# zhangganlin/vista-slam

Hardware: AMD Instinct MI355X
Metric: STA image-pairs/sec @512x384 (higher is better)
Workload: dtype f16x3-split MFMA (3 fp16 products) in the transformer and the pose head; fp16 MFMA + one block-scaled fp8 correction MFMA in the DPT head's convolutions; fp32 accumulate; 1 GPU; 512x384 batch=8 pairs/GPU STA two-view forward (BASELINE configs[1]); pairs_per_gpu=8, H=384, W=512, precision=f16x3h, parallelism=single GPU

## Files before the change

vista_slam_amd/csrc/gemm2.h:

```cpp
#pragma once
#include "gemm.h"
#include <type_traits>

typedef short short8 __attribute__((ext_vector_type(8)));

__device__ __forceinline__ void glds16(const void* gsrc, void* lds_dst_wave_base) {
    __builtin_amdgcn_global_load_lds((const __attribute__((address_space(1))) void*)gsrc,
                                     (__attribute__((address_space(3))) void*)lds_dst_wave_base, 16, 0, 0);
}

template <bool SPLIT, int BM, int BN>
constexpr int gemm2_smem_bytes(int nstg = 2) { return nstg * (SPLIT ? 2 : 1) * (BM + BN) * 64; }

template <bool SPLIT>
__device__ __forceinline__ int lds2_off(int row, int chunk) {
    return SPLIT ? row * 128 + ((chunk ^ ((row >> 1) & 7)) << 4) : row * 64 + ((chunk ^ ((row >> 2) & 3)) << 4);
}

template <int BM, int MT, int NT, int WM, int WAVES_N>
__device__ __forceinline__ void head_epilogue(const GemmParams& p, const floatx16 (&acc)[MT][NT], int64_t pix_base, int rstride, int rows_valid,
                                              int cols_valid, int wm, int wn, int tid, char* smem) {
    float* red = reinterpret_cast<float*>(smem);
    const int lane = tid & 63, l31 = lane & 31, lhi = lane >> 5;
    float bv[NT], w4[NT][4];
#pragma unroll
    for (int j = 0; j < NT; ++j) {
        const int col = (wn * NT + j) * 32 + l31;
        bv[j] = p.bias ? p.bias[col] : 0.f;
#pragma unroll
        for (int o = 0; o < 4; ++o) w4[j][o] = p.hw4[o * 128 + col];
    }
    __syncthreads();
#pragma unroll
    for (int i = 0; i < MT; ++i) {
        float part[64];
#pragma unroll
        for (int r = 0; r < 16; ++r) {
#pragma unroll
            for (int j = 0; j < NT; ++j) {
                const float v = fmaxf(acc[i][j][r] + bv[j], 0.f);
#pragma unroll
                for (int o = 0; o < 4; ++o) part[r * 4 + o] = j == 0 ? v * w4[j][o] : __builtin_fmaf(v, w4[j][o], part[r * 4 + o]);
            }
        }
#pragma unroll
        for (int m = 16, n = 64; m >= 1; m >>= 1, n >>= 1) {
            const bool up = (l31 & m) != 0;
#pragma unroll
            for (int k = 0; k < 32; ++k) {
                if (k < n / 2) {
                    const float send = up ? part[k] : part[k + n / 2];
                    const float keep = up ? part[k + n / 2] : part[k];
                    part[k] = keep + __shfl_xor(send, m);
                }
            }
        }
        const int r = l31 >> 1, row = wm * WM + i * 32 + (r & 3) + 8 * (r >> 2) + 4 * lhi;
        *reinterpret_cast<float2*>(red + ((size_t)wn * BM + row) * 4 + (l31 & 1) * 2) = make_float2(part[0], part[1]);
    }
    __syncthreads();
    if (tid < BM) {
        const int64_t pix = pix_base + (int64_t)(tid >> 5) * rstride + (tid & 31);
        if (pix < p.M && (tid >> 5) < rows_valid && (tid & 31) < cols_valid) {
            float4 a = *reinterpret_cast<const float4*>(red + (size_t)tid * 4);
#pragma unroll
            for (int w = 1; w < WAVES_N; ++w) {
                const float4 b = *reinterpret_cast<const float4*>(red + ((size_t)w * BM + tid) * 4);
                a.x += b.x; a.y += b.y; a.z += b.z; a.w += b.w;
            }
            const float x = a.x + p.hb4[0], y = a.y + p.hb4[1], z = a.z + p.hb4[2], c = a.w + p.hb4[3];
            const float d = sqrtf(x * x + y * y + z * z);
            const float sc = expm1f(d) / fmaxf(d, 1e-8f);
            const bool second = pix >= p.hsplit;
            const int64_t q = second ? pix - p.hsplit : pix;
            float* pts = (second ? p.hptsB : p.hptsA) + q * 3;
            pts[0] = x * sc; pts[1] = y * sc; pts[2] = z * sc;
            (second ? p.hconfB : p.hconfA)[q] = 1.0f + expf(c);
        }
    }
}

template <int BM, int MT, int WM, int WAVES_N>
__device__ __forceinline__ void head_epilogue_t(const GemmParams& p, const floatx16 (&acc)[MT][1], int64_t pix_base, int rstride, int rows_valid,
                                                int cols_valid, int wm, int wn, int tid, char* smem) {
    float* red = reinterpret_cast<float*>(smem);
    const int lane = tid & 63, l31 = lane & 31, lhi = lane >> 5;
    float bv[16];
#pragma unroll
    for (int r = 0; r < 16; ++r) bv[r] = p.bias ? p.bias[wn * 32 + (r & 3) + 8 * (r >> 2) + 4 * lhi] : 0.f;
    half8 wh[2], wl[2];
    {
        RangeAcc rw;
#pragma unroll
        for (int w = 0; w < 2; ++w)
#pragma unroll
            for (int e = 0; e < 8; ++e) {
                const float x = l31 < 4 ? p.hw4[l31 * 128 + wn * 32 + 16 * w + 8 * lhi + e] * p.hw4_scale[l31 & 3] : 0.f;
                f16 h_, l_; split_f16(x, h_, l_, rw);
                wh[w][e] = h_; wl[w][e] = l_;
            }
    }
    __syncthreads();
    RangeAcc ra;
#pragma unroll
    for (int i = 0; i < MT; ++i) {
        floatx16 o;
#pragma unroll
        for (int r = 0; r < 16; ++r) o[r] = 0.f;
#pragma unroll
        for (int w = 0; w < 2; ++w) {
            union { half8 h; unsigned u[4]; } ph, pl;
#pragma unroll
            for (int e = 0; e < 8; ++e) {
                const float v = fmaxf(acc[i][0][8 * w + e] + bv[8 * w + e], 0.f);
                f16 h_, l_; split_f16(v, h_, l_, ra);
                ph.h[e] = h_; pl.h[e] = l_;
            }
#pragma unroll
            for (int e = 0; e < 2; ++e) {
                auto r1 = __builtin_amdgcn_permlane32_swap(ph.u[e], ph.u[2 + e], false, false);
                ph.u[e] = r1[0]; ph.u[2 + e] = r1[1];
                auto r2 = __builtin_amdgcn_permlane32_swap(pl.u[e], pl.u[2 + e], false, false);
                pl.u[e] = r2[0]; pl.u[2 + e] = r2[1];
            }
            o = __builtin_amdgcn_mfma_f32_32x32x16_f16(wl[w], ph.h, o, 0, 0, 0);
            o = __builtin_amdgcn_mfma_f32_32x32x16_f16(wh[w], pl.h, o, 0, 0, 0);
            o = __builtin_amdgcn_mfma_f32_32x32x16_f16(wh[w], ph.h, o, 0, 0, 0);
        }
        if (lhi == 0) *reinterpret_cast<float4*>(red + ((size_t)wn * BM + wm * WM + i * 32 + l31) * 4) =
            make_float4(o[0] / p.hw4_scale[0], o[1] / p.hw4_scale[1], o[2] / p.hw4_scale[2], o[3] / p.hw4_scale[3]);
    }
    ra.flush(p.range);
    __syncthreads();
    if (tid < BM) {
        const int64_t pix = pix_base + (int64_t)(tid >> 5) * rstride + (tid & 31);
        if (pix < p.M && (tid >> 5) < rows_valid && (tid & 31) < cols_valid) {
            float4 a = *reinterpret_cast<const float4*>(red + (size_t)tid * 4);
#pragma unroll
            for (int w = 1; w < WAVES_N; ++w) {
                const float4 b = *reinterpret_cast<const float4*>(red + ((size_t)w * BM + tid) * 4);
                a.x += b.x; a.y += b.y; a.z += b.z; a.w += b.w;
            }
            const float x = a.x + p.hb4[0], y = a.y + p.hb4[1], z = a.z + p.hb4[2], c = a.w + p.hb4[3];
            const float d = sqrtf(x * x + y * y + z * z);
            const float sc = expm1f(d) / fmaxf(d, 1e-8f);
            const bool second = pix >= p.hsplit;
            const int64_t q = second ? pix - p.hsplit : pix;
            float* pts = (second ? p.hptsB : p.hptsA) + q * 3;
            pts[0] = x * sc; pts[1] = y * sc; pts[2] = z * sc;
            (second ? p.hconfB : p.hconfA)[q] = 1.0f + expf(c);
        }
    }
}

template <bool SPLIT, int EPI, int NW, bool MX = false>
__device__ __forceinline__ void gemm2_tail(const GemmParams& p, const int tb, char* smem) {
    const int tid = threadIdx.x, lane = tid & 63, l31 = lane & 31, lhi = lane >> 5;
    const int wave = __builtin_amdgcn_readfirstlane(tid >> 6);
    constexpr int A_ES = SPLIT ? 64 : 32;
    const int row0 = p.M - p.m_tail, col0 = tb * 32;
    const int arow = row0 + l31 < p.M ? row0 + l31 : p.M - 1;
    const int brow = col0 + l31 < p.N ? col0 + l31 : p.N - 1;
    const f16* ap = p.A_hi + (size_t)arow * A_ES + lhi * 8;
    const f16* bp = p.B_hi + (size_t)brow * 64 + lhi * 8;
    const size_t a_kstride = (size_t)p.a_rp * A_ES, b_kstride = (size_t)p.N * 64;
    const int nkt_all = p.K / GEMM_BK;
    const int kt0 = (int)((int64_t)wave * nkt_all / NW), kt1 = (int)((int64_t)(wave + 1) * nkt_all / NW);
    struct Frag { uint4 ah[2], al[2], bh[2], bl[2]; };
    auto load = [&](int kt, Frag& f) {
        const f16* a = ap + kt * a_kstride;
        const f16* b = bp + kt * b_kstride;
#pragma unroll
        for (int ks = 0; ks < 2; ++ks) {
            f.ah[ks] = ldg16(a + ks * 16); f.bh[ks] = ldg16(b + ks * 16);
            if (MX) {
                f.al[ks] = ldg16(a - lhi * 8 + 32 + lhi * 16 + ks * 8); f.bl[ks] = ldg16(b - lhi * 8 + 32 + lhi * 16 + ks * 8);
            } else if (SPLIT) { f.al[ks] = ldg16(a + 32 + ks * 16); f.bl[ks] = ldg16(b + 32 + ks * 16); }
        }
    };
    floatx16 acc;
#pragma unroll
    for (int r = 0; r < 16; ++r) acc[r] = 0.f;
    auto mma = [&](const Frag& f) {
        if constexpr (MX) {
            typedef int int8v __attribute__((ext_vector_type(8)));
            union U8 { struct { uint4 x, y; } q; int8v v; } a8, b8;
#pragma unroll
            for (int ks = 0; ks < 2; ++ks) {
                H8 ah, bh; ah.u = f.ah[ks]; bh.u = f.bh[ks];
                acc = __builtin_amdgcn_mfma_f32_32x32x16_f16(ah.h, bh.h, acc, 0, 0, 0);
            }
            a8.q.x = f.al[0]; a8.q.y = f.al[1]; b8.q.x = f.bl[0]; b8.q.y = f.bl[1];
            constexpr int sc_a = 127 - STA_MX_A_SLO, sc_b = 127 - STA_MX_W_SHI;
            acc = __builtin_amdgcn_mfma_scale_f32_32x32x64_f8f6f4(a8.v, b8.v, acc, 1 , 0 , 0, sc_a, 0, sc_b);
            return;
        }
#pragma unroll
        for (int ks = 0; ks < 2; ++ks) {
            H8 ah, al, bh, bl; ah.u = f.ah[ks]; bh.u = f.bh[ks];
            if (SPLIT) {
                al.u = f.al[ks]; bl.u = f.bl[ks];
                acc = __builtin_amdgcn_mfma_f32_32x32x16_f16(al.h, bh.h, acc, 0, 0, 0);
                acc = __builtin_amdgcn_mfma_f32_32x32x16_f16(ah.h, bl.h, acc, 0, 0, 0);
            }
            acc = __builtin_amdgcn_mfma_f32_32x32x16_f16(ah.h, bh.h, acc, 0, 0, 0);
        }
    };
#pragma unroll 1
    for (int kt = kt0; kt < kt1; ++kt) {
        Frag f;
        load(kt, f);
        mma(f);
    }
    float* red = reinterpret_cast<float*>(smem);
#pragma unroll
    for (int r = 0; r < 16; ++r) red[(wave * 16 + r) * 64 + lane] = acc[r];
    __syncthreads();
    if (wave != 0) return;
#pragma unroll 1
    for (int w = 1; w < NW; ++w) {
#pragma unroll
        for (int r = 0; r < 16; ++r) acc[r] += red[(w * 16 + r) * 64 + lane];
    }
    epilogue_tile<SPLIT, EPI>(p, acc, row0, col0 + l31, lane, 0);
}

#ifndef STA_RING_ABL
#define STA_RING_ABL 0
#endif
template <bool SPLIT, int AMODE, int EPI, int BM, int BN, int WAVES_M, int WAVES_N, int ABL_ = 0, int NSTG = 2, bool MX = false>
__device__ __forceinline__ void gemm2_body(const GemmParams& p, const int block_id_in) {
    constexpr int ABL = ABL_ | (NSTG > 2 ? STA_RING_ABL : 0);
    extern __shared__ __attribute__((aligned(16))) char smem[];
    constexpr int NW = WAVES_M * WAVES_N;
    constexpr int WM = BM / WAVES_M, WN = BN / WAVES_N, MT = WM / 32, NT = WN / 32;
    constexpr int RB = SPLIT ? 128 : 64;
    constexpr int RPS = 1024 / RB;
    constexpr int CPR = RB / 16;
    constexpr int A_TILE = BM * RB, B_TILE = BN * RB, STAGE = A_TILE + B_TILE;
    constexpr int NSA = BM / RPS, NSB = BN / RPS;
    constexpr int SA = (NSA + NW - 1) / NW, SB = (NSB + NW - 1) / NW;
    constexpr int A_ES = SPLIT ? 64 : 32;
    static_assert(BM % 32 == 0 && BN % 32 == 0 && WM % 32 == 0 && WN % 32 == 0, "tile/wave mismatch");
    constexpr bool TRN = EPI == EPI_HEAD && BN == 128 && NT == 1;

    int block_id = block_id_in;
    constexpr bool HAS_TAIL = AMODE == A_DENSE && NSTG == 2 && ABL_ == 0 && BM >= 192 &&
                              (EPI == EPI_F32 || EPI == EPI_F32R || ((EPI == EPI_GELU || EPI == EPI_QKV) && !MX));
    if constexpr (HAS_TAIL) {
        if (p.m_tail > 0) {
            const int ntail = (p.N + 31) >> 5;
            if (block_id < ntail) { gemm2_tail<SPLIT, EPI, NW, MX>(p, block_id, smem); return; }
            block_id -= ntail;
        }
    }
    const int tid = threadIdx.x, lane = tid & 63;
    const int wave = __builtin_amdgcn_readfirstlane(tid >> 6);
    const int wm = wave / WAVES_N, wn = wave % WAVES_N;
    const int l31 = lane & 31, lhi = lane >> 5;
    unsigned long long clk0 = 0, rt0 = 0;
    if (p.clk_dbg) { clk0 = __builtin_readcyclecounter(); rt0 = __builtin_amdgcn_s_memrealtime(); }
    unsigned long long st0 = 0, st1 = 0, st2 = 0;
    if (p.stamps) st0 = __builtin_amdgcn_s_memrealtime();

    const int tiles_m = (p.M - (HAS_TAIL ? p.m_tail : 0) + BM - 1) / BM, tiles_n = (p.N + BN - 1) / BN;
    const int ksplit = p.ksplit > 1 ? p.ksplit : 1;
    const int nwg = tiles_m * tiles_n * ksplit;
    int t;
    {
        const int bid = block_id, q = nwg / 8, r = nwg % 8, xcd = bid % 8;
        t = (xcd < r ? xcd * (q + 1) : r * (q + 1) + (xcd - r) * q) + bid / 8;
    }
    const int kslice = t % ksplit;
    t /= ksplit;
    int bm, bn;
    {
        const int band = t / (4 * tiles_n);
        const int hb = tiles_m - band * 4 < 4 ? tiles_m - band * 4 : 4;
        const int local = t - band * 4 * tiles_n;
        bm = band * 4 + local % hb;
        bn = local / hb;
    }
    const int m0 = bm * BM, n0 = bn * BN;

    const int row_in = lane / CPR, c_lds = lane % CPR;
    unsigned a_src[SA], b_src[SB];
    int cv_pix0[SA]; unsigned cv_mask[SA], cv_coff[SA];
#pragma unroll
    for (int s = 0; s < SA; ++s) {
        const int row = RPS * (wave + NW * s) + row_in;
        const int sw = SPLIT ? (row >> 1) & 7 : (row >> 2) & 3;
        const int chunk = c_lds ^ sw;
        const int gm = m0 + row;
        if (AMODE == A_DENSE) {
            const int gmc = gm < p.M ? gm : p.M - 1;
            a_src[s] = ((unsigned)gmc * A_ES + chunk * 8) * 2u;
        } else {
            const bool rok = gm < p.M;
            const int gmc = rok ? gm : 0;
            const int hw = p.Ho * p.Wo;
            const int img = gmc / hw;
            const int rem = gmc - img * hw;
            const int y0 = (rem / p.Wo) * p.cstride - 1, x0 = (rem % p.Wo) * p.cstride - 1;
            cv_pix0[s] = (img * p.Hi + y0) * p.Wi + x0;
            unsigned mk = 0;
#pragma unroll
            for (int t = 0; t < 9; ++t) {
                const int yi = y0 + t / 3, xi = x0 + t % 3;
                if (rok && yi >= 0 && yi < p.Hi && xi >= 0 && xi < p.Wi) mk |= 1u << t;
            }
            cv_mask[s] = mk;
            cv_coff[s] = (unsigned)chunk * 16u;
            a_src[s] = 0;
        }
    }
#pragma unroll
    for (int s = 0; s < SB; ++s) {
        const int row = RPS * (wave + NW * s) + row_in;
        const int sw = SPLIT ? (row >> 1) & 7 : (row >> 2) & 3;
        const int gn = n0 + row;
        const int gnc = gn < p.N ? gn : p.N - 1;
        b_src[s] = ((unsigned)gnc * 64 + (c_lds ^ sw) * 8) * 2u;
    }
    const size_t a_kstride = (size_t)p.a_rp * A_ES, b_kstride = (size_t)p.N * 64;

    int cv_tap = 0, cv_cb = 0;
    const char* a_run = nullptr; const char* b_run = nullptr;
    auto issue_tile = [&](int kt, int stage) {
        char* sA = smem + stage * STAGE;
        char* sB = sA + A_TILE;
        int tap_off = 0; const char* a_cb = nullptr;
        if (AMODE == A_CONV3) {
            const int ky = cv_tap >= 6 ? 2 : (cv_tap >= 3 ? 1 : 0), kx = cv_tap - 3 * ky;
            tap_off = ky * p.Wi + kx;
            a_cb = reinterpret_cast<const char*>(p.A_hi) + (size_t)cv_cb * p.a_rp * (A_ES * 2);
        }
#pragma unroll
        for (int s = 0; s < SA; ++s) {
            if (NSA % NW != 0 && wave + NW * s >= NSA) continue;
            char* dst = sA + (wave + NW * s) * 1024;
            if (AMODE == A_DENSE) {
                unsigned o = a_src[s];
                asm volatile("" : "+v"(o));
                glds16(a_run + o, dst);
            } else {
                const unsigned off = (unsigned)(cv_pix0[s] + tap_off) * (unsigned)(A_ES * 2) + cv_coff[s];
                const bool ok = (cv_mask[s] >> cv_tap) & 1u;
                glds16(ok ? static_cast<const void*>(a_cb + off) : static_cast<const void*>(p.zero_page), dst);
            }
        }
        if (AMODE == A_CONV3) { if (++cv_cb == (p.Cin >> 5)) { cv_cb = 0; ++cv_tap; } }
#pragma unroll
        for (int s = 0; s < SB; ++s) {
            if (NSB % NW != 0 && wave + NW * s >= NSB) continue;
            unsigned o = b_src[s];
            asm volatile("" : "+v"(o));
            glds16(b_run + o, sB + (wave + NW * s) * 1024);
        }
        a_run += a_kstride * 2; b_run += b_kstride * 2;
    };

    floatx16 acc[MT][NT];
#pragma unroll
    for (int i = 0; i < MT; ++i)
#pragma unroll
        for (int j = 0; j < NT; ++j)
#pragma unroll
            for (int r = 0; r < 16; ++r) acc[i][j][r] = 0.f;

    const int nkt_all = p.K / GEMM_BK;
    const int kt0 = (int)((int64_t)kslice * nkt_all / ksplit);
    const int nkt = (int)((int64_t)(kslice + 1) * nkt_all / ksplit) - kt0;
    if (AMODE == A_CONV3) { const int cblocks = p.Cin >> 5; cv_tap = kt0 / cblocks; cv_cb = kt0 - cv_tap * cblocks; }
    a_run = reinterpret_cast<const char*>(p.A_hi + kt0 * a_kstride); b_run = reinterpret_cast<const char*>(p.B_hi + kt0 * b_kstride);
    constexpr bool RING = NSTG > 2;
    constexpr int GPW = SA + SB;
    static_assert(!RING || (NSA % NW == 0 && NSB % NW == 0), "ring needs the same DMA count in every wave");
    static_assert(NSTG >= 2 && NSTG <= 5, "2..5 stages");
    if (RING) {
#pragma unroll
        for (int s0 = 0; s0 < NSTG - 1; ++s0)
            if (s0 < nkt && !(ABL & 1)) issue_tile(kt0 + s0, s0);
    } else {
        issue_tile(kt0, 0);
        asm volatile("s_waitcnt vmcnt(0)" ::: "memory");
        __syncthreads();
        if (p.stamps) st1 = __builtin_amdgcn_s_memrealtime();
    }

    const bool late_dma = (ABL & 8) && !RING && wave >= NW / 2;
    auto compute_tile = [&](const int cur, const int kt, auto relu_c) {
        constexpr bool RELU = AMODE == A_CONV3 && decltype(relu_c)::value;
        const char* sA = smem + cur * STAGE;
        const char* sB = sA + A_TILE;
        if (MX) {
            typedef int int4v __attribute__((ext_vector_type(4)));
            typedef int int8v __attribute__((ext_vector_type(8)));
            half8 ah[MT], bh[NT];
#pragma unroll
            for (int ks = 0; ks < 2; ++ks) {
                const int chunk = ks * 2 + lhi;
#pragma unroll
                for (int i = 0; i < MT; ++i) {
                    ah[i] = *reinterpret_cast<const half8*>(sA + lds2_off<true>(wm * WM + i * 32 + l31, chunk));
                    if (RELU) {
                        union { half8 h; unsigned u[4]; } t; t.h = ah[i];
#pragma unroll
                        for (int w = 0; w < 4; ++w) { const unsigned sgn = (t.u[w] >> 15) & 0x00010001u; t.u[w] &= ~((sgn << 16) - sgn); }
                        ah[i] = t.h;
                    }
                }
#pragma unroll
                for (int j = 0; j < NT; ++j) bh[j] = *reinterpret_cast<const half8*>(sB + lds2_off<true>(wn * WN + j * 32 + l31, chunk));
#pragma unroll
                for (int i = 0; i < MT; ++i)
#pragma unroll
                    for (int j = 0; j < NT; ++j)
                        acc[i][j] = TRN ? __builtin_amdgcn_mfma_f32_32x32x16_f16(bh[j], ah[i], acc[i][j], 0, 0, 0)
                                        : __builtin_amdgcn_mfma_f32_32x32x16_f16(ah[i], bh[j], acc[i][j], 0, 0, 0);
            }
            union U8 { struct { int4v x, y; } q; int8v v; };
            U8 a8[MT], b8[NT];
#pragma unroll
            for (int i = 0; i < MT; ++i) {
                const int ra = wm * WM + i * 32 + l31;
                a8[i].q.x = *reinterpret_cast<const int4v*>(sA + lds2_off<true>(ra, 4 + 2 * lhi));
                a8[i].q.y = *reinterpret_cast<const int4v*>(sA + lds2_off<true>(ra, 5 + 2 * lhi));
                if (RELU) {
#pragma unroll
                    for (int w = 0; w < 8; ++w) { const unsigned u = (unsigned)a8[i].v[w]; const unsigned sgn = (u >> 7) & 0x00010001u; a8[i].v[w] = (int)(u & ~((sgn << 16) - sgn)); }
                }
            }
#pragma unroll
            for (int j = 0; j < NT; ++j) {
                const int rb = wn * WN + j * 32 + l31;
                b8[j].q.x = *reinterpret_cast<const int4v*>(sB + lds2_off<true>(rb, 4 + 2 * lhi));
                b8[j].q.y = *reinterpret_cast<const int4v*>(sB + lds2_off<true>(rb, 5 + 2 * lhi));
            }
            constexpr int sc_a = 127 - STA_MX_A_SLO, sc_b = 127 - STA_MX_W_SHI;
#pragma unroll
            for (int i = 0; i < MT; ++i)
#pragma unroll
                for (int j = 0; j < NT; ++j)
                    acc[i][j] = TRN ? __builtin_amdgcn_mfma_scale_f32_32x32x64_f8f6f4(b8[j].v, a8[i].v, acc[i][j], 0 , 1 , 0, sc_b, 0, sc_a)
                                    : __builtin_amdgcn_mfma_scale_f32_32x32x64_f8f6f4(a8[i].v, b8[j].v, acc[i][j], 1 , 0 , 0, sc_a, 0, sc_b);
            return;
        }
        half8 a_hi[MT], a_lo[MT], b_hi[NT], b_lo[NT];
        if (ABL & 2) {
#pragma unroll
            for (int i = 0; i < MT; ++i) { a_hi[i] = (half8)(f16)(0.001f * (lane + i)); a_lo[i] = a_hi[i]; asm volatile("" : "+v"(a_hi[i]), "+v"(a_lo[i])); }
#pragma unroll
            for (int j = 0; j < NT; ++j) { b_hi[j] = (half8)(f16)(0.002f * (lane + j)); b_lo[j] = b_hi[j]; asm volatile("" : "+v"(b_hi[j]), "+v"(b_lo[j])); }
        }
#pragma unroll
        for (int ks = 0; ks < 2; ++ks) {
            const int chunk = ks * 2 + lhi;
#pragma unroll
            for (int i = 0; i < MT && !(ABL & 2); ++i) {
                const int ra = wm * WM + i * 32 + l31;
                a_hi[i] = *reinterpret_cast<const half8*>(sA + lds2_off<SPLIT>(ra, chunk));
                if (SPLIT) a_lo[i] = *reinterpret_cast<const half8*>(sA + lds2_off<SPLIT>(ra, 4 + chunk));
                if (AMODE == A_CONV3) {
                    if (RELU) {
                        union { half8 h; unsigned u[4]; } ah, al;
                        ah.h = a_hi[i]; al.h = a_lo[i];
#pragma unroll
                        for (int w = 0; w < 4; ++w) {
                            const unsigned sgn = (ah.u[w] >> 15) & 0x00010001u;
                            const unsigned m = (sgn << 16) - sgn;
                            ah.u[w] &= ~m;
                            if (SPLIT) al.u[w] &= ~m;
                        }
                        a_hi[i] = ah.h; if (SPLIT) a_lo[i] = al.h;
                    }
                }
            }
#pragma unroll
            for (int j = 0; j < NT && !(ABL & 2); ++j) {
                const int rb = wn * WN + j * 32 + l31;
                b_hi[j] = *reinterpret_cast<const half8*>(sB + lds2_off<SPLIT>(rb, chunk));
                if (SPLIT) b_lo[j] = *reinterpret_cast<const half8*>(sB + lds2_off<SPLIT>(rb, 4 + chunk));
            }
            if (ABL & 4) {
#pragma unroll
                for (int i = 0; i < MT; ++i) asm volatile("" ::"v"(a_hi[i]), "v"(a_lo[i]));
#pragma unroll
                for (int j = 0; j < NT; ++j) asm volatile("" ::"v"(b_hi[j]), "v"(b_lo[j]));
                continue;
            }
            if (SPLIT && (ABL & 16)) {
                if (ks == 1) {
                    typedef int int8v __attribute__((ext_vector_type(8)));
#pragma unroll
                    for (int i = 0; i < MT; ++i)
#pragma unroll
                        for (int j = 0; j < NT; ++j) {
                            union { struct { half8 x, y; } h; int8v v; } ua, ub;
                            ua.h.x = a_lo[i]; ua.h.y = a_hi[i]; ub.h.x = b_hi[j]; ub.h.y = b_lo[j];
                            acc[i][j] = __builtin_amdgcn_mfma_scale_f32_32x32x64_f8f6f4(ua.v, ub.v, acc[i][j], 0, 0, 0, 0x7f, 0, 0x7f);
                        }
                }
            } else if (SPLIT) {
#pragma unroll
                for (int i = 0; i < MT; ++i)
#pragma unroll
                    for (int j = 0; j < NT; ++j)
                        acc[i][j] = TRN ? __builtin_amdgcn_mfma_f32_32x32x16_f16(b_hi[j], a_lo[i], acc[i][j], 0, 0, 0) : __builtin_amdgcn_mfma_f32_32x32x16_f16(a_lo[i], b_hi[j], acc[i][j], 0, 0, 0);
#pragma unroll
                for (int i = 0; i < MT; ++i)
#pragma unroll
                    for (int j = 0; j < NT; ++j)
                        acc[i][j] = TRN ? __builtin_amdgcn_mfma_f32_32x32x16_f16(b_lo[j], a_hi[i], acc[i][j], 0, 0, 0) : __builtin_amdgcn_mfma_f32_32x32x16_f16(a_hi[i], b_lo[j], acc[i][j], 0, 0, 0);
            }
#pragma unroll
            for (int i = 0; i < MT; ++i)
#pragma unroll
                for (int j = 0; j < NT; ++j)
                    acc[i][j] = TRN ? __builtin_amdgcn_mfma_f32_32x32x16_f16(b_hi[j], a_hi[i], acc[i][j], 0, 0, 0) : __builtin_amdgcn_mfma_f32_32x32x16_f16(a_hi[i], b_hi[j], acc[i][j], 0, 0, 0);
            if ((ABL & 8) && ks == 0 && late_dma && kt + 1 < nkt) issue_tile(kt0 + kt + 1, cur ^ 1);
        }
    };
    auto main_loop = [&](auto relu_c) {
    if (RING) {
        int cur = 0, nxt = NSTG - 1, kt = 0;
        for (; kt + NSTG - 1 < nkt; ++kt) {
            asm volatile("s_waitcnt vmcnt(%0)\n\ts_barrier" ::"n"((NSTG - 2) * GPW) : "memory");
            if (p.stamps && kt == 0) st1 = __builtin_amdgcn_s_memrealtime();
            if (!(ABL & 1)) issue_tile(kt0 + kt + NSTG - 1, nxt);
            compute_tile(cur, kt, relu_c);
            cur = cur + 1 == NSTG ? 0 : cur + 1;
            nxt = nxt + 1 == NSTG ? 0 : nxt + 1;
        }
        for (; kt < nkt; ++kt) {
            const int rem = nkt - 1 - kt;
            if (rem == 0) asm volatile("s_waitcnt vmcnt(0)\n\ts_barrier" ::: "memory");
            else if (rem == 1) asm volatile("s_waitcnt vmcnt(%0)\n\ts_barrier" ::"n"(GPW) : "memory");
            else if (rem == 2) asm volatile("s_waitcnt vmcnt(%0)\n\ts_barrier" ::"n"(2 * GPW) : "memory");
            else asm volatile("s_waitcnt vmcnt(%0)\n\ts_barrier" ::"n"(3 * GPW) : "memory");
            if (p.stamps && kt == 0) st1 = __builtin_amdgcn_s_memrealtime();
            compute_tile(cur, kt, relu_c);
            cur = cur + 1 == NSTG ? 0 : cur + 1;
        }
    } else {
        for (int kt = 0; kt < nkt; ++kt) {
            const int cur = kt & 1;
            if (kt + 1 < nkt && !(ABL & 1) && !late_dma) issue_tile(kt0 + kt + 1, cur ^ 1);
            compute_tile(cur, kt, relu_c);
            asm volatile("s_waitcnt vmcnt(0)" ::: "memory");
            __syncthreads();
        }
    }
    };
    if constexpr (AMODE == A_CONV3) {
        if (p.relu_in) main_loop(std::integral_constant<bool, true>{});
        else main_loop(std::integral_constant<bool, false>{});
    } else main_loop(std::integral_constant<bool, false>{});

    if (p.stamps) {
        asm volatile("" ::"v"(acc[MT - 1][NT - 1][15]), "v"(acc[0][0][0]) : "memory");
        st2 = __builtin_amdgcn_s_memrealtime();
    }
    if constexpr (EPI == EPI_HEAD) {
        if constexpr (BN == 128) {
            if constexpr (TRN) head_epilogue_t<BM, MT, WM, WAVES_N>(p, acc, m0, 32, BM / 32, 32, wm, wn, tid, smem);
            else head_epilogue<BM, MT, NT, WM, WAVES_N>(p, acc, m0, 32, BM / 32, 32, wm, wn, tid, smem);
        }
    } else {
        char* const wave_lds = ((EPI == EPI_QKV || EPI == EPI_GELU || EPI == EPI_F16) && NW * EPI_LDS_BYTES <= NSTG * STAGE) ? smem + wave * EPI_LDS_BYTES : nullptr;
        if (RING && wave_lds != nullptr) __syncthreads();
#pragma unroll
        for (int j = 0; j < NT; ++j)
#pragma unroll
            for (int i = 0; i < MT; ++i)
                { epilogue_tile<SPLIT, EPI>(p, acc[i][j], m0 + wm * WM + i * 32, n0 + wn * WN + j * 32 + l31, lane, kslice, -1, wave_lds); if (EPI == EPI_F16 || EPI == EPI_CONVT) STA_EPI_TILE_FENCE(); }
    }
    if (p.stamps) {
        asm volatile("s_waitcnt vmcnt(0)" ::: "memory");
        if (tid == 0 && block_id_in < 2048) {
            unsigned long long* o = p.stamps + (size_t)block_id_in * 4;
            o[0] = st0; o[1] = st1; o[2] = st2; o[3] = __builtin_amdgcn_s_memrealtime();
        }
    }
    if (p.clk_dbg && tid == 0 && (block_id & 63) == 0) {
        atomicAdd(p.clk_dbg, __builtin_readcyclecounter() - clk0);
        atomicAdd(p.clk_dbg + 1, __builtin_amdgcn_s_memrealtime() - rt0);
    }
}

template <bool SPLIT, int AMODE, int EPI, int BM, int BN, int WAVES_M, int WAVES_N, int ABL = 0, int NSTG = 2, bool MX = false>
__global__ __launch_bounds__(WAVES_M* WAVES_N * 64) void gemm2_kernel(const GemmParams p) {
    gemm2_body<SPLIT, AMODE, EPI, BM, BN, WAVES_M, WAVES_N, ABL, NSTG, MX>(p, blockIdx.x);
}

template <bool SPLIT, int AMODE, int EPI, int BM, int BN, int WAVES_M, int WAVES_N>
__global__ __launch_bounds__(WAVES_M* WAVES_N * 64) void gemm2_pair_kernel(const GemmParams pa, const GemmParams pb, const int tiles_a) {
    if ((int)blockIdx.x < tiles_a) gemm2_body<SPLIT, AMODE, EPI, BM, BN, WAVES_M, WAVES_N>(pa, blockIdx.x);
    else gemm2_body<SPLIT, AMODE, EPI, BM, BN, WAVES_M, WAVES_N>(pb, blockIdx.x - tiles_a);
}
```

vista_slam_amd/csrc/sta_bench.inc:

```

extern "C" double sta_flops_per_pair(const sta_handle* h, int H, int W) {
    if (!h) return 0;
    const sta_config& c = h->cfg;
    const double E = c.enc_embed_dim, D = c.dec_embed_dim, R = c.mlp_ratio;
    const double hp = H / 16, wp = W / 16, N = hp * wp, Np = N + 1;
    double f_enc = 2 * N * 768 * E + c.enc_depth * ((8 + 4 * R) * N * E * E + 4 * N * N * E);
    double f_dec = 4 * N * E * D + 2.0 * c.dec_depth * ((16 + 4 * R) * Np * D * D + 8 * Np * Np * D);
    auto conv = [](double hh, double ww, double ci, double co, double k) { return 2.0 * hh * ww * ci * co * k * k; };
    double h3 = floor((hp - 1) / 2) + 1, w3 = floor((wp - 1) / 2) + 1;
    double f = 0;
    f += conv(hp, wp, E, 96, 1) + 2.0 * hp * wp * 96 * 96 * 16;
    f += conv(hp, wp, D, 192, 1) + 2.0 * hp * wp * 192 * 192 * 4;
    f += conv(hp, wp, D, 384, 1);
    f += conv(hp, wp, D, 768, 1) + conv(h3, w3, 768, 768, 3);
    f += conv(4 * hp, 4 * wp, 96, 256, 3) + conv(2 * hp, 2 * wp, 192, 256, 3) + conv(hp, wp, 384, 256, 3) + conv(h3, w3, 768, 256, 3);
    f += 2 * conv(h3, w3, 256, 256, 3) + conv(hp, wp, 256, 256, 1);
    f += 4 * conv(hp, wp, 256, 256, 3) + conv(2 * hp, 2 * wp, 256, 256, 1);
    f += 4 * conv(2 * hp, 2 * wp, 256, 256, 3) + conv(4 * hp, 4 * wp, 256, 256, 1);
    f += 4 * conv(4 * hp, 4 * wp, 256, 256, 3) + conv(8 * hp, 8 * wp, 256, 256, 1);
    f += conv(8 * hp, 8 * wp, 256, 128, 3) + conv(16 * hp, 16 * wp, 128, 128, 3) + conv(16 * hp, 16 * wp, 128, 4, 1);
    double f_pose = 2.0 * (D * 512 + 2 * 512 * 512 + 512 * 13);
    return 2 * f_enc + f_dec + 2 * f + 2 * f_pose;
}

#ifdef STA_TEST_HOOKS

__global__ void fill_rand_f16_kernel(f16* p, int64_t n, uint32_t seed, float scale) {
    int64_t i = (int64_t)blockIdx.x * blockDim.x + threadIdx.x;
    const int64_t step = (int64_t)gridDim.x * blockDim.x;
    for (; i < n; i += step) {
        uint32_t x = (uint32_t)i * 0x9E3779B1u + seed;
        x ^= x >> 16; x *= 0x85EBCA6Bu; x ^= x >> 13; x *= 0xC2B2AE35u; x ^= x >> 16;
        p[i] = (f16)(((float)(x >> 8) * (2.0f / 16777216.0f) - 1.0f) * scale);
    }
}

template <int BM, int BN, int WMS, int WNS, int ABL>
static int bench_launch2(bool split, const GemmParams& p, hipStream_t st) {
    if (split) {
        constexpr int smem = gemm2_smem_bytes<true, BM, BN>();
        HIPCHK(hipFuncSetAttribute((const void*)gemm2_kernel<true, A_DENSE, EPI_F32, BM, BN, WMS, WNS, ABL>, hipFuncAttributeMaxDynamicSharedMemorySize, smem));
        hipLaunchKernelGGL((gemm2_kernel<true, A_DENSE, EPI_F32, BM, BN, WMS, WNS, ABL>), dim3((unsigned)(((p.M + BM - 1) / BM) * ((p.N + BN - 1) / BN))), dim3(WMS * WNS * 64), smem, st, p);
    } else {
#ifndef STA_DEV_FAST
        constexpr int smem = gemm2_smem_bytes<false, BM, BN>();
        HIPCHK(hipFuncSetAttribute((const void*)gemm2_kernel<false, A_DENSE, EPI_F32, BM, BN, WMS, WNS, ABL>, hipFuncAttributeMaxDynamicSharedMemorySize, smem));
        hipLaunchKernelGGL((gemm2_kernel<false, A_DENSE, EPI_F32, BM, BN, WMS, WNS, ABL>), dim3((unsigned)(((p.M + BM - 1) / BM) * ((p.N + BN - 1) / BN))), dim3(WMS * WNS * 64), smem, st, p);
#else
        return set_err("development build: precision f16 kernels are not compiled in");
#endif
    }
    return 0;
}

static float g_bench_ghz = 0.f;
extern "C" float sta_bench_gemm_last_ghz() { return g_bench_ghz; }

extern "C" int sta_bench_gemm(sta_handle* h, int M, int N, int K, int iters, int tile, int abl, float* ms_out, void* stream) {
    REQUIRE(h && ms_out && iters > 0, "bad argument");
    DEV_SCOPE(h->device);
    hipStream_t st = (hipStream_t)stream;
    const bool split = h->prec != STA_PREC_F16;
    int64_t bytes = ((int64_t)M * K + (int64_t)N * K) * 4 + (int64_t)M * N * 4 + N * 4 + (1 << 16);
    CHK(ensure_ws(h, bytes, st));
    h->dry = false;
    Bump ws = cur_bump(h);
    Planes A = ws.act(M, K, true);
    Lin Wt; Wt.N = N; Wt.K = K; Wt.w = ws.act(N, K, true);
    Wt.bias = (float*)ws.take((int64_t)N * 4);
    float* C = (float*)ws.take((int64_t)M * N * 4);
    unsigned long long* clk = (unsigned long long*)ws.take(16);
    REQUIRE(!ws.overflow, "internal: bench workspace overflow");
    hipLaunchKernelGGL(fill_rand_f16_kernel, dim3(2048), dim3(256), 0, st, A.hi, (int64_t)M * K * 2, 1u, 1.0f);
    hipLaunchKernelGGL(fill_rand_f16_kernel, dim3(2048), dim3(256), 0, st, Wt.w.hi, (int64_t)N * K * 2, 3u, 0.03f);
    HIPCHK(hipMemsetAsync(Wt.bias, 0, (size_t)N * 4, st));
    if (!split) { A.lo = nullptr; }
    GemmParams p = gp_dense(A, K, Wt, M);
    p.range = h->range;
    p.C32 = C; p.ldc = N; p.ldr = N; p.zero_page = h->zero_page;
    const int keep = h->gemm_variant;
    auto once = [&]() -> int {
#ifdef STA_BENCH_EXPERIMENTS
        if (tile >= 2 && abl > 0) {
            if (tile == 2) {
                switch (abl) {
                    case 1: return bench_launch2<256, 256, 2, 4, 1>(split, p, st);
                    case 2: return bench_launch2<256, 256, 2, 4, 2>(split, p, st);
                    case 3: return bench_launch2<256, 256, 2, 4, 3>(split, p, st);
                    case 4: return bench_launch2<256, 256, 2, 4, 4>(split, p, st);
                    case 5: return bench_launch2<256, 256, 2, 4, 5>(split, p, st);
                    case 6: return bench_launch2<256, 256, 2, 4, 6>(split, p, st);
                    default: return bench_launch2<256, 256, 2, 4, 7>(split, p, st);
                }
            }
            switch (abl) {
                case 1: return bench_launch2<192, 128, 2, 4, 1>(split, p, st);
                case 2: return bench_launch2<192, 128, 2, 4, 2>(split, p, st);
                case 3: return bench_launch2<192, 128, 2, 4, 3>(split, p, st);
                case 4: return bench_launch2<192, 128, 2, 4, 4>(split, p, st);
                case 5: return bench_launch2<192, 128, 2, 4, 5>(split, p, st);
                case 6: return bench_launch2<192, 128, 2, 4, 6>(split, p, st);
                default: return bench_launch2<192, 128, 2, 4, 7>(split, p, st);
            }
        }
#else
        if (abl > 0) return set_err("bench: main-loop ablations need a library built with -DSTA_BENCH_EXPERIMENTS");
#endif
        if (tile >= 100) {
            GemmParams q = p; q.resid = q.C32; q.ldr = q.ldc;
            switch (tile - 100) {
                case 6: return bench_launch2<192, 128, 2, 4, 0>(split, q, st);
                case 21: return bench_launch2<256, 256, 4, 4, 0>(split, q, st);
                case 22: return bench_launch2<192, 256, 3, 4, 0>(split, q, st);
#ifdef STA_BENCH_EXPERIMENTS
                case 2: return bench_launch2<256, 256, 2, 4, 0>(split, q, st);
                case 20: return bench_launch2<192, 128, 3, 2, 0>(split, q, st);
                case 23: return bench_launch2<128, 256, 2, 4, 0>(split, q, st);
                case 25: return bench_launch2<192, 96, 2, 3, 0>(split, q, st);
                case 26: return bench_launch2<384, 128, 4, 2, 0>(split, q, st);
#endif
                default: return set_err("bench: unknown residual tile %d", tile);
            }
        }
        if (tile == 21) return bench_launch2<256, 256, 4, 4, 0>(split, p, st);
        if (tile == 22) return bench_launch2<192, 256, 3, 4, 0>(split, p, st);
        if (tile == 6) return bench_launch2<192, 128, 2, 4, 0>(split, p, st);
#ifdef STA_BENCH_EXPERIMENTS
        if (tile == 16) { GemmParams q = p; q.mx = 1; return launch_gemm2<true, A_DENSE, EPI_F32, 192, 128, 2, 4, 2, true>(q, st); }
        if (tile == 17) { GemmParams q = p; q.mx = 1; q.resid = q.C32; q.ldr = q.ldc; return launch_gemm2<true, A_DENSE, EPI_F32, 192, 128, 2, 4, 2, true>(q, st); }
        if (tile == 20) return bench_launch2<192, 128, 3, 2, 0>(split, p, st);
        if (tile == 23) return bench_launch2<128, 256, 2, 4, 0>(split, p, st);
        if (tile == 25) return bench_launch2<192, 96, 2, 3, 0>(split, p, st);
        if (tile == 26) return bench_launch2<384, 128, 4, 2, 0>(split, p, st);
        if (tile == 2) return bench_launch2<256, 256, 2, 4, 0>(split, p, st);
        if (tile == 3) return bench_launch2<256, 128, 4, 2, 0>(split, p, st);
        if (tile == 10) return split ? launch_gemm2<true, A_DENSE, EPI_F32, 256, 128, 4, 2, 3>(p, st)
                                     : launch_gemm2<false, A_DENSE, EPI_F32, 256, 128, 4, 2, 3>(p, st);
        if (tile == 14) return bench_launch2<256, 256, 2, 4, 16>(split, p, st);
        if (tile == 15) return bench_launch2<192, 128, 2, 4, 16>(split, p, st);
        if (tile == 11) return bench_launch2<256, 256, 2, 4, 8>(split, p, st);
        if (tile == 12) return bench_launch2<192, 128, 2, 4, 8>(split, p, st);
        if (tile == 5) return bench_launch2<192, 256, 2, 4, 0>(split, p, st);
        if (tile == 13) { GemmParams q = p; q.resid = q.C32; q.ldr = q.ldc; return bench_launch2<192, 128, 2, 4, 0>(split, q, st); }
        if (tile == 7) return bench_launch2<192, 128, 2, 2, 0>(split, p, st);
        if (tile == 8) return bench_launch2<128, 192, 2, 2, 0>(split, p, st);
        if (tile == 9) return bench_launch2<128, 128, 2, 2, 0>(split, p, st);
#else
        if (tile > 1) return set_err("bench: tile %d is an experiment (build with -DSTA_BENCH_EXPERIMENTS); product tiles: 0 auto, 1, 6, 21, 22, +100 = in-place residual", tile);
#endif
        h->gemm_variant = tile == 1 ? 1 : 0;
        int r = launch_gemm<A_DENSE, EPI_F32>(h, p, st);
        h->gemm_variant = keep;
        return r;
    };
    hipEvent_t e0, e1;
    HIPCHK(hipEventCreate(&e0)); HIPCHK(hipEventCreate(&e1));
    for (int i = 0; i < 2; ++i) CHK(once());
    HIPCHK(hipEventRecord(e0, st));
    for (int i = 0; i < iters; ++i) CHK(once());
    HIPCHK(hipEventRecord(e1, st));
    HIPCHK(hipEventSynchronize(e1));
    HIPCHK(hipGetLastError());
    float ms = 0; HIPCHK(hipEventElapsedTime(&ms, e0, e1));
    *ms_out = ms / iters;
    HIPCHK(hipMemsetAsync(clk, 0, 16, st));
    p.clk_dbg = clk;
    for (int i = 0; i < 3; ++i) CHK(once());
    p.clk_dbg = nullptr;
    unsigned long long hc[2] = {0, 0};
    HIPCHK(hipMemcpyAsync(hc, clk, 16, hipMemcpyDeviceToHost, st));
    HIPCHK(hipStreamSynchronize(st));
    g_bench_ghz = hc[1] ? (float)((double)hc[0] / ((double)hc[1] / 100e6) * 1e-9) : 0.f;
    hipEventDestroy(e0); hipEventDestroy(e1);
    return 0;
}


extern "C" int sta_bench_gemm_stamps(sta_handle* h, int M, int N, int K, int resid, double* out, unsigned long long* raw, int raw_cap, void* stream) {
    REQUIRE(h && out && M > 0 && N > 0 && K > 0, "bad argument");
    DEV_SCOPE(h->device);
    hipStream_t st = (hipStream_t)stream;
    int64_t bytes = ((int64_t)M * K + (int64_t)N * K) * 4 + (int64_t)M * N * 4 + N * 4 + (int64_t)8192 * 32 + (1 << 16);
    CHK(ensure_ws(h, bytes, st));
    h->dry = false;
    Bump ws = cur_bump(h);
    Planes A = ws.act(M, K, true);
    Lin Wt; Wt.N = N; Wt.K = K; Wt.w = ws.act(N, K, true);
    Wt.bias = (float*)ws.take((int64_t)N * 4);
    float* C = (float*)ws.take((int64_t)M * N * 4);
    const int cap = 8192;
    unsigned long long* stamps = (unsigned long long*)ws.take((int64_t)cap * 32);
    REQUIRE(!ws.overflow && h->prec != STA_PREC_F16, "internal: bench workspace overflow / f16x3 only");
    hipLaunchKernelGGL(fill_rand_f16_kernel, dim3(2048), dim3(256), 0, st, A.hi, (int64_t)M * K * 2, 1u, 1.0f);
    hipLaunchKernelGGL(fill_rand_f16_kernel, dim3(2048), dim3(256), 0, st, Wt.w.hi, (int64_t)N * K * 2, 3u, 0.03f);
    HIPCHK(hipMemsetAsync(Wt.bias, 0, (size_t)N * 4, st));
    HIPCHK(hipMemsetAsync(C, 0, (size_t)M * N * 4, st));
    GemmParams p = gp_dense(A, K, Wt, M);
    p.range = h->range;
    p.C32 = C; p.ldc = N; p.ldr = N; p.zero_page = h->zero_page;
    if (resid) { p.resid = C; p.slab = h->cur->slab; }
    int ks = 0;
    auto launch = [&](GemmParams& q) -> int {
        if (resid == 2 && !small_grid(h, M, N)) { q.slab = nullptr; return launch_gemm<A_DENSE, EPI_F32R>(h, q, st, &ks); }
        return launch_gemm<A_DENSE, EPI_F32>(h, q, st, &ks);
    };
    hipEvent_t e0, e1;
    HIPCHK(hipEventCreate(&e0)); HIPCHK(hipEventCreate(&e1));
    for (int i = 0; i < 3; ++i) CHK(launch(p));
    HIPCHK(hipMemsetAsync(stamps, 0, (size_t)cap * 32, st));
    p.stamps = stamps;
    CHK(launch(p));
    HIPCHK(hipMemsetAsync(stamps, 0, (size_t)cap * 32, st));
    HIPCHK(hipStreamSynchronize(st));
    HIPCHK(hipEventRecord(e0, st));
    CHK(launch(p));
    HIPCHK(hipEventRecord(e1, st));
    HIPCHK(hipEventSynchronize(e1));
    float ms = 0; HIPCHK(hipEventElapsedTime(&ms, e0, e1));
    std::vector<unsigned long long> hs((size_t)cap * 4);
    HIPCHK(hipMemcpy(hs.data(), stamps, (size_t)cap * 32, hipMemcpyDeviceToHost));
    hipEventDestroy(e0); hipEventDestroy(e1);
    if (raw) memcpy(raw, hs.data(), (size_t)(raw_cap < cap ? raw_cap : cap) * 32);
    std::vector<double> pro, loop, epi, whole;
    unsigned long long t0min = ~0ull, t0max = 0, t3min = ~0ull, t3max = 0;
    for (int b = 0; b < cap; ++b) {
        const unsigned long long* q = &hs[(size_t)b * 4];
        if (!q[3]) continue;
        pro.push_back((double)(q[1] - q[0]) * 0.01); loop.push_back((double)(q[2] - q[1]) * 0.01); epi.push_back((double)(q[3] - q[2]) * 0.01);
        whole.push_back((double)(q[3] - q[0]) * 0.01);
        if (q[0] < t0min) t0min = q[0]; if (q[0] > t0max) t0max = q[0];
        if (q[3] < t3min) t3min = q[3]; if (q[3] > t3max) t3max = q[3];
    }
    REQUIRE(!pro.empty(), "no stamps recorded (this shape did not run on a gemm2 family)");
    auto med = [](std::vector<double>& v) { std::sort(v.begin(), v.end()); return v[v.size() / 2]; };
    out[0] = (double)pro.size(); out[1] = (double)(t3max - t0min) * 0.01; out[2] = med(pro); out[3] = med(loop); out[4] = med(epi);
    out[5] = (double)(t0max - t0min) * 0.01; out[6] = (double)(t3max - t3min) * 0.01; out[7] = ms * 1e3; out[8] = ks; out[9] = med(whole);
    return 0;
}

extern "C" int sta_bench_attention(sta_handle* h, int S, int heads, int nq, int nk, int pose, int iters, int which, float* ms_out, void* stream) {
    REQUIRE(h && ms_out && iters > 0 && S > 0 && heads > 0 && nq > 0 && nk > 0, "bad argument");
    DEV_SCOPE(h->device);
    hipStream_t st = (hipStream_t)stream;
    const bool split = h->prec != STA_PREC_F16;
    const int nmax = (nq > nk ? nq : nk) + (pose ? 1 : 0), npad = rup(nmax, 64);
    const int64_t hsz = (int64_t)S * heads * npad * 64, M = (int64_t)S * nq + (pose ? S : 0);
    CHK(ensure_ws(h, (3 * hsz + M * heads * 64) * 4 + (1 << 16), st));
    h->dry = false;
    Bump ws = cur_bump(h);
    QKVOut o; o.npad = npad; o.q = ws.planes(hsz, true); o.k = ws.planes(hsz, true); o.vt = ws.planes(hsz, true);
    Planes ao = ws.act(M, heads * 64, true);
    REQUIRE(!ws.overflow, "internal: bench workspace overflow");
    if (!split) { o.q.lo = o.k.lo = o.vt.lo = nullptr; ao.lo = nullptr; }
    hipLaunchKernelGGL(fill_rand_f16_kernel, dim3(2048), dim3(256), 0, st, o.q.hi, hsz * 2, 5u, 1.0f);
    hipLaunchKernelGGL(fill_rand_f16_kernel, dim3(2048), dim3(256), 0, st, o.k.hi, hsz * 2, 7u, 1.0f);
    hipLaunchKernelGGL(fill_rand_f16_kernel, dim3(2048), dim3(256), 0, st, o.vt.hi, hsz * 2, 9u, 1.0f);
    REQUIRE(which == 0, "sta_bench_attention: no alternative kernel in this build");
    hipEvent_t e0, e1;
    HIPCHK(hipEventCreate(&e0)); HIPCHK(hipEventCreate(&e1));
    int rc = 0;
    for (int i = 0; i < 2 && rc == 0; ++i) rc = run_attn(h, o, ao, heads * 64, S, heads, nq, nk, 0, st, pose != 0);
    HIPCHK(hipEventRecord(e0, st));
    for (int i = 0; i < iters && rc == 0; ++i) rc = run_attn(h, o, ao, heads * 64, S, heads, nq, nk, 0, st, pose != 0);
    HIPCHK(hipEventRecord(e1, st));
    if (rc != 0) return rc;
    HIPCHK(hipEventSynchronize(e1));
    float ms = 0; HIPCHK(hipEventElapsedTime(&ms, e0, e1));
    *ms_out = ms / iters;
    hipEventDestroy(e0); hipEventDestroy(e1);
    return 0;
}
#endif
```

Before: 182.5 pairs/s.

## Switch non-MX GEMM inner loop to 16x16x32 MFMA with permlane remap

```diff
diff --git a/vista_slam_amd/csrc/gemm2.h b/vista_slam_amd/csrc/gemm2.h
--- a/vista_slam_amd/csrc/gemm2.h
+++ b/vista_slam_amd/csrc/gemm2.h
@@ -258,6 +258,8 @@
     const int wave = __builtin_amdgcn_readfirstlane(tid >> 6);
     const int wm = wave / WAVES_N, wn = wave % WAVES_N;
     const int l31 = lane & 31, lhi = lane >> 5;
+    const int m16 = lane & 15, g16 = lane >> 4;
+    const int a_perm = (m16 & 3) | ((m16 & 4) << 1) | ((m16 & 8) >> 1);
     unsigned long long clk0 = 0, rt0 = 0;
     if (p.clk_dbg) { clk0 = __builtin_readcyclecounter(); rt0 = __builtin_amdgcn_s_memrealtime(); }
     unsigned long long st0 = 0, st1 = 0, st2 = 0;
@@ -367,6 +369,14 @@
         for (int j = 0; j < NT; ++j)
 #pragma unroll
             for (int r = 0; r < 16; ++r) acc[i][j][r] = 0.f;
+    constexpr bool ACC16 = !MX && !TRN;
+    floatx4 acc4[ACC16 ? MT : 1][ACC16 ? NT : 1][2][2];
+#pragma unroll
+    for (int i = 0; i < (ACC16 ? MT : 1); ++i)
+#pragma unroll
+        for (int j = 0; j < (ACC16 ? NT : 1); ++j)
+#pragma unroll
+            for (int b = 0; b < 4; ++b) acc4[i][j][b >> 1][b & 1] = floatx4{0.f, 0.f, 0.f, 0.f};
 
     const int nkt_all = p.K / GEMM_BK;
     const int kt0 = (int)((int64_t)kslice * nkt_all / ksplit);
@@ -389,11 +399,23 @@
     }
 
     const bool late_dma = (ABL & 8) && !RING && wave >= NW / 2;
+    auto relu_frag = [](half8& hi, half8& lo) {
+        union { half8 h; unsigned u[4]; } ah, al;
+        ah.h = hi; al.h = lo;
+#pragma unroll
+        for (int w = 0; w < 4; ++w) {
+            const unsigned sgn = (ah.u[w] >> 15) & 0x00010001u;
+            const unsigned m = (sgn << 16) - sgn;
+            ah.u[w] &= ~m;
+            if (SPLIT) al.u[w] &= ~m;
+        }
+        hi = ah.h; if (SPLIT) lo = al.h;
+    };
     auto compute_tile = [&](const int cur, const int kt, auto relu_c) {
         constexpr bool RELU = AMODE == A_CONV3 && decltype(relu_c)::value;
         const char* sA = smem + cur * STAGE;
         const char* sB = sA + A_TILE;
-        if (MX) {
+        if constexpr (MX) {
             typedef int int4v __attribute__((ext_vector_type(4)));
             typedef int int8v __attribute__((ext_vector_type(8)));
             half8 ah[MT], bh[NT];
@@ -444,81 +466,99 @@
                 for (int j = 0; j < NT; ++j)
                     acc[i][j] = TRN ? __builtin_amdgcn_mfma_scale_f32_32x32x64_f8f6f4(b8[j].v, a8[i].v, acc[i][j], 0 , 1 , 0, sc_b, 0, sc_a)
                                     : __builtin_amdgcn_mfma_scale_f32_32x32x64_f8f6f4(a8[i].v, b8[j].v, acc[i][j], 1 , 0 , 0, sc_a, 0, sc_b);
-            return;
-        }
-        half8 a_hi[MT], a_lo[MT], b_hi[NT], b_lo[NT];
+        } else if constexpr (TRN) {
+            half8 a_hi[MT], a_lo[MT], b_hi[NT], b_lo[NT];
+#pragma unroll
+            for (int ks = 0; ks < 2; ++ks) {
+                const int chunk = ks * 2 + lhi;
+#pragma unroll
+                for (int i = 0; i < MT; ++i) {
+                    const int ra = wm * WM + i * 32 + l31;
+                    a_hi[i] = *reinterpret_cast<const half8*>(sA + lds2_off<SPLIT>(ra, chunk));
+                    if (SPLIT) a_lo[i] = *reinterpret_cast<const half8*>(sA + lds2_off<SPLIT>(ra, 4 + chunk));
+                    if (RELU) relu_frag(a_hi[i], a_lo[i]);
+                }
+#pragma unroll
+                for (int j = 0; j < NT; ++j) {
+                    const int rb = wn * WN + j * 32 + l31;
+                    b_hi[j] = *reinterpret_cast<const half8*>(sB + lds2_off<SPLIT>(rb, chunk));
+                    if (SPLIT) b_lo[j] = *reinterpret_cast<const half8*>(sB + lds2_off<SPLIT>(rb, 4 + chunk));
+                }
+                if (SPLIT) {
+#pragma unroll
+                    for (int i = 0; i < MT; ++i)
+#pragma unroll
+                        for (int j = 0; j < NT; ++j) acc[i][j] = __builtin_amdgcn_mfma_f32_32x32x16_f16(b_hi[j], a_lo[i], acc[i][j], 0, 0, 0);
+#pragma unroll
+                    for (int i = 0; i < MT; ++i)
+#pragma unroll
+                        for (int j = 0; j < NT; ++j) acc[i][j] = __builtin_amdgcn_mfma_f32_32x32x16_f16(b_lo[j], a_hi[i], acc[i][j], 0, 0, 0);
+                }
+#pragma unroll
+                for (int i = 0; i < MT; ++i)
+#pragma unroll
+                    for (int j = 0; j < NT; ++j) acc[i][j] = __builtin_amdgcn_mfma_f32_32x32x16_f16(b_hi[j], a_hi[i], acc[i][j], 0, 0, 0);
+            }
+        } else {
+        half8 b_hi[NT][2], b_lo[NT][2];
         if (ABL & 2) {
 #pragma unroll
-            for (int i = 0; i < MT; ++i) { a_hi[i] = (half8)(f16)(0.001f * (lane + i)); a_lo[i] = a_hi[i]; asm volatile("" : "+v"(a_hi[i]), "+v"(a_lo[i])); }
-#pragma unroll
-            for (int j = 0; j < NT; ++j) { b_hi[j] = (half8)(f16)(0.002f * (lane + j)); b_lo[j] = b_hi[j]; asm volatile("" : "+v"(b_hi[j]), "+v"(b_lo[j])); }
-        }
-#pragma unroll
-        for (int ks = 0; ks < 2; ++ks) {
-            const int chunk = ks * 2 + lhi;
-#pragma unroll
-            for (int i = 0; i < MT && !(ABL & 2); ++i) {
-                const int ra = wm * WM + i * 32 + l31;
-                a_hi[i] = *reinterpret_cast<const half8*>(sA + lds2_off<SPLIT>(ra, chunk));
-                if (SPLIT) a_lo[i] = *reinterpret_cast<const half8*>(sA + lds2_off<SPLIT>(ra, 4 + chunk));
-                if (AMODE == A_CONV3) {
-                    if (RELU) {
-                        union { half8 h; unsigned u[4]; } ah, al;
-                        ah.h = a_hi[i]; al.h = a_lo[i];
-#pragma unroll
-                        for (int w = 0; w < 4; ++w) {
-                            const unsigned sgn = (ah.u[w] >> 15) & 0x00010001u;
-                            const unsigned m = (sgn << 16) - sgn;
-                            ah.u[w] &= ~m;
-                            if (SPLIT) al.u[w] &= ~m;
-                        }
-                        a_hi[i] = ah.h; if (SPLIT) a_lo[i] = al.h;
+            for (int j = 0; j < NT; ++j)
+#pragma unroll
+                for (int bj = 0; bj < 2; ++bj) {
+                    b_hi[j][bj] = (half8)(f16)(0.002f * (lane + 2 * j + bj)); b_lo[j][bj] = b_hi[j][bj];
+                    asm volatile("" : "+v"(b_hi[j][bj]), "+v"(b_lo[j][bj]));
+                }
+        } else {
+#pragma unroll
+            for (int j = 0; j < NT; ++j)
+#pragma unroll
+                for (int bj = 0; bj < 2; ++bj) {
+                    const int rb = wn * WN + j * 32 + bj * 16 + m16;
+                    b_hi[j][bj] = *reinterpret_cast<const half8*>(sB + lds2_off<SPLIT>(rb, g16));
+                    if (SPLIT) b_lo[j][bj] = *reinterpret_cast<const half8*>(sB + lds2_off<SPLIT>(rb, 4 + g16));
+                }
+        }
+#pragma unroll
+        for (int i = 0; i < MT; ++i)
+#pragma unroll
+            for (int bi = 0; bi < 2; ++bi) {
+                half8 a_hi, a_lo;
+                if (ABL & 2) {
+                    a_hi = (half8)(f16)(0.001f * (lane + 2 * i + bi)); a_lo = a_hi;
+                    asm volatile("" : "+v"(a_hi), "+v"(a_lo));
+                } else {
+                    const int ra = wm * WM + i * 32 + bi * 16 + a_perm;
+                    a_hi = *reinterpret_cast<const half8*>(sA + lds2_off<SPLIT>(ra, g16));
+                    if (SPLIT) a_lo = *reinterpret_cast<const half8*>(sA + lds2_off<SPLIT>(ra, 4 + g16));
+                    if (RELU) relu_frag(a_hi, a_lo);
+                }
+                if (ABL & 4) {
+                    asm volatile("" ::"v"(a_hi), "v"(a_lo));
+                } else {
+                    if (SPLIT) {
+#pragma unroll
+                        for (int j = 0; j < NT; ++j)
+#pragma unroll
+                            for (int bj = 0; bj < 2; ++bj) acc4[i][j][bi][bj] = __builtin_amdgcn_mfma_f32_16x16x32_f16(a_lo, b_hi[j][bj], acc4[i][j][bi][bj], 0, 0, 0);
+#pragma unroll
+                        for (int j = 0; j < NT; ++j)
+#pragma unroll
+                            for (int bj = 0; bj < 2; ++bj) acc4[i][j][bi][bj] = __builtin_amdgcn_mfma_f32_16x16x32_f16(a_hi, b_lo[j][bj], acc4[i][j][bi][bj], 0, 0, 0);
                     }
-                }
-            }
-#pragma unroll
-            for (int j = 0; j < NT && !(ABL & 2); ++j) {
-                const int rb = wn * WN + j * 32 + l31;
-                b_hi[j] = *reinterpret_cast<const half8*>(sB + lds2_off<SPLIT>(rb, chunk));
-                if (SPLIT) b_lo[j] = *reinterpret_cast<const half8*>(sB + lds2_off<SPLIT>(rb, 4 + chunk));
-            }
-            if (ABL & 4) {
-#pragma unroll
-                for (int i = 0; i < MT; ++i) asm volatile("" ::"v"(a_hi[i]), "v"(a_lo[i]));
-#pragma unroll
-                for (int j = 0; j < NT; ++j) asm volatile("" ::"v"(b_hi[j]), "v"(b_lo[j]));
-                continue;
-            }
-            if (SPLIT && (ABL & 16)) {
-                if (ks == 1) {
-                    typedef int int8v __attribute__((ext_vector_type(8)));
-#pragma unroll
-                    for (int i = 0; i < MT; ++i)
-#pragma unroll
-                        for (int j = 0; j < NT; ++j) {
-                            union { struct { half8 x, y; } h; int8v v; } ua, ub;
-                            ua.h.x = a_lo[i]; ua.h.y = a_hi[i]; ub.h.x = b_hi[j]; ub.h.y = b_lo[j];
-                            acc[i][j] = __builtin_amdgcn_mfma_scale_f32_32x32x64_f8f6f4(ua.v, ub.v, acc[i][j], 0, 0, 0, 0x7f, 0, 0x7f);
-                        }
-                }
-            } else if (SPLIT) {
-#pragma unroll
-                for (int i = 0; i < MT; ++i)
 #pragma unroll
                     for (int j = 0; j < NT; ++j)
-                        acc[i][j] = TRN ? __builtin_amdgcn_mfma_f32_32x32x16_f16(b_hi[j], a_lo[i], acc[i][j], 0, 0, 0) : __builtin_amdgcn_mfma_f32_32x32x16_f16(a_lo[i], b_hi[j], acc[i][j], 0, 0, 0);
-#pragma unroll
-                for (int i = 0; i < MT; ++i)
-#pragma unroll
-                    for (int j = 0; j < NT; ++j)
-                        acc[i][j] = TRN ? __builtin_amdgcn_mfma_f32_32x32x16_f16(b_lo[j], a_hi[i], acc[i][j], 0, 0, 0) : __builtin_amdgcn_mfma_f32_32x32x16_f16(a_hi[i], b_lo[j], acc[i][j], 0, 0, 0);
-            }
-#pragma unroll
-            for (int i = 0; i < MT; ++i)
-#pragma unroll
-                for (int j = 0; j < NT; ++j)
-                    acc[i][j] = TRN ? __builtin_amdgcn_mfma_f32_32x32x16_f16(b_hi[j], a_hi[i], acc[i][j], 0, 0, 0) : __builtin_amdgcn_mfma_f32_32x32x16_f16(a_hi[i], b_hi[j], acc[i][j], 0, 0, 0);
-            if ((ABL & 8) && ks == 0 && late_dma && kt + 1 < nkt) issue_tile(kt0 + kt + 1, cur ^ 1);
+#pragma unroll
+                        for (int bj = 0; bj < 2; ++bj) acc4[i][j][bi][bj] = __builtin_amdgcn_mfma_f32_16x16x32_f16(a_hi, b_hi[j][bj], acc4[i][j][bi][bj], 0, 0, 0);
+                }
+                if ((ABL & 8) && 2 * i + bi == MT - 1 && late_dma && kt + 1 < nkt) issue_tile(kt0 + kt + 1, cur ^ 1);
+            }
+        if (ABL & 4) {
+#pragma unroll
+            for (int j = 0; j < NT; ++j)
+#pragma unroll
+                for (int bj = 0; bj < 2; ++bj) asm volatile("" ::"v"(b_hi[j][bj]), "v"(b_lo[j][bj]));
+        }
         }
     };
     auto main_loop = [&](auto relu_c) {
@@ -557,6 +597,20 @@
         else main_loop(std::integral_constant<bool, false>{});
     } else main_loop(std::integral_constant<bool, false>{});
 
+    if constexpr (ACC16) {
+#pragma unroll
+        for (int i = 0; i < MT; ++i)
+#pragma unroll
+            for (int j = 0; j < NT; ++j)
+#pragma unroll
+                for (int bi = 0; bi < 2; ++bi)
+#pragma unroll
+                    for (int q = 0; q < 4; ++q) {
+                        const auto xy = __builtin_amdgcn_permlane16_swap(__float_as_uint(acc4[i][j][bi][0][q]), __float_as_uint(acc4[i][j][bi][1][q]), false, false);
+                        acc[i][j][8 * bi + q] = __uint_as_float(xy[0]);
+                        acc[i][j][8 * bi + 4 + q] = __uint_as_float(xy[1]);
+                    }
+    }
     if (p.stamps) {
         asm volatile("" ::"v"(acc[MT - 1][NT - 1][15]), "v"(acc[0][0][0]) : "memory");
         st2 = __builtin_amdgcn_s_memrealtime();
diff --git a/vista_slam_amd/csrc/sta_bench.inc b/vista_slam_amd/csrc/sta_bench.inc
--- a/vista_slam_amd/csrc/sta_bench.inc
+++ b/vista_slam_amd/csrc/sta_bench.inc
@@ -136,8 +136,6 @@
         if (tile == 3) return bench_launch2<256, 128, 4, 2, 0>(split, p, st);
         if (tile == 10) return split ? launch_gemm2<true, A_DENSE, EPI_F32, 256, 128, 4, 2, 3>(p, st)
                                      : launch_gemm2<false, A_DENSE, EPI_F32, 256, 128, 4, 2, 3>(p, st);
-        if (tile == 14) return bench_launch2<256, 256, 2, 4, 16>(split, p, st);
-        if (tile == 15) return bench_launch2<192, 128, 2, 4, 16>(split, p, st);
         if (tile == 11) return bench_launch2<256, 256, 2, 4, 8>(split, p, st);
         if (tile == 12) return bench_launch2<192, 128, 2, 4, 8>(split, p, st);
         if (tile == 5) return bench_launch2<192, 256, 2, 4, 0>(split, p, st);
```

Result: faster. 191.3 pairs/s, median of 6 (+4.8%).
